# google/sbsim

Hardware: AMD Instinct MI355X
Metric: zone-updates/sec (env-steps/sec x 9 zones) at batch=64k buildings per GPU (higher is better)
Workload: dtype f64

## Files before the change

sbsim_amd/csrc/step_roll.hip:

```cpp
#include "step_roll_cfg.h"
#include "sweep_common.h"

namespace sb {
namespace {

using namespace sweep;
using namespace roll;

#ifndef SB_ONE_WAIT
#define SB_ONE_WAIT 1
#endif
constexpr int kWin = 63;
constexpr int kTS = 32;
constexpr int kSeamPad = 8;

struct PairBuf {
  d2 ud0, lr0, ud1, lr1;
  d2 A;
  d2 sm;
};

struct Acc {
  double cur;
  double neg;
  int sg;
  int tr, fin;
  double sre, sro;
};


template <int NR>
struct Ctx {
  const double *Arow;
  const double *Aext;
  const double *seam;
  const unsigned long long *cw;
  unsigned long long w, wn;
#ifdef SB_EXP_NOCOEF
  d2 kc;
#endif
};

template <int NR, int S>
__device__ __forceinline__ lds_d2 step_set(Ctx<NR> &x) {
  constexpr int j = S % NR;
  static_assert(NR % 8 == 0, "whole class words per period");
  if constexpr (j % 8 == 0) {
    x.w = x.wn;
    x.wn = x.cw[((j / 8 + 1) % (NR / 8)) * 64];
  }
  const unsigned h = j % 8 < 4 ? (unsigned)x.w : (unsigned)(x.w >> 32);
  unsigned off;
  if constexpr (j % 4 == 0) asm("v_lshlrev_b32_sdwa %0, 5, %1 dst_sel:DWORD dst_unused:UNUSED_PAD src0_sel:DWORD src1_sel:BYTE_0" : "=v"(off) : "v"(h));
  else if constexpr (j % 4 == 1) asm("v_lshlrev_b32_sdwa %0, 5, %1 dst_sel:DWORD dst_unused:UNUSED_PAD src0_sel:DWORD src1_sel:BYTE_1" : "=v"(off) : "v"(h));
  else if constexpr (j % 4 == 2) asm("v_lshlrev_b32_sdwa %0, 5, %1 dst_sel:DWORD dst_unused:UNUSED_PAD src0_sel:DWORD src1_sel:BYTE_2" : "=v"(off) : "v"(h));
  else asm("v_lshlrev_b32_sdwa %0, 5, %1 dst_sel:DWORD dst_unused:UNUSED_PAD src0_sel:DWORD src1_sel:BYTE_3" : "=v"(off) : "v"(h));
  return (lds_d2)off;
}

template <int NR, int S, bool SEAM, int NAR>
__device__ __forceinline__ void load_first(PairBuf &p, Ctx<NR> &x, const double (&Areg)[NAR]) {
#ifdef SB_EXP_NOCOEF
  p.ud0 = p.lr0 = x.kc;
  const lds_d2 ct = nullptr;
#else
  const lds_d2 ct = step_set<NR, S>(x);
  p.ud0 = ct[0];
#endif
#if defined(SB_EXP_ONECOEF)
  p.lr0 = p.ud0;
#elif !defined(SB_EXP_NOCOEF)
  p.lr0 = ct[1];
#endif
  constexpr int q = (S + 1) % NR, NL = lds_slots(NR), AS = a_stride(NR);
  static_assert(q % 2 == 0 && AS % 2 == 0, "pairs start at odd steps");
  if constexpr (q < AS) p.A = *(const d2 *)(x.Arow + q);
  else if constexpr (q < NL) p.A = *(const d2 *)(x.Aext + (q - AS));
  else p.A = d2{Areg[q - NL], Areg[q + 1 - NL]};
  if constexpr (SEAM && S >= kWin) p.sm = *(const d2 *)(x.seam + S);
  else p.sm = d2{0.0, 0.0};
}
template <int NR, int S>
__device__ __forceinline__ void load_second(PairBuf &p, Ctx<NR> &x) {
#ifdef SB_EXP_NOCOEF
  p.ud1 = p.lr1 = x.kc;
#else
  const lds_d2 ct = step_set<NR, S>(x);
  p.ud1 = ct[0];
#ifdef SB_EXP_ONECOEF
  p.lr1 = p.ud1;
#else
  p.lr1 = ct[1];
#endif
#endif
}

__device__ __forceinline__ void track(Acc &acc, double d) {
#ifdef SB_EXP_NOTRACK
  return;
#endif
  asm("v_max_f32 %0, %0, %1" : "+v"(acc.fin) : "v"(acc.tr));
  asm("v_max_f32_dpp %0, %0, |%1| wave_shr:1 row_mask:0xf bank_mask:0xf bound_ctrl:1" : "+v"(acc.tr) : "v"(__double2hiint(d)));
}

template <int NR, int S, bool EXACT, bool FREE = false>
__device__ __forceinline__ void step(double (&e)[NR], double (&bk)[kWin], d2 ud, d2 lr, double A,
                                     double sm, Acc &acc) {
  static_assert(S >= kWin, "the ramp-up has a step of its own: step_ramp");
  static_assert(!FREE || !EXACT, "free periods: the library's kernel");
  constexpr int r = S % NR, rm = (S + NR - 1) % NR, rp = (S + 1) % NR;
  const double Dn = wave_shift1<0x130, true>(e[rp], sm);
  double t;
  asm("v_fma_f64 %0, %1, %2, %3" : "=&v"(t) : "v"(ud.y), "v"(Dn), "v"(A));
  t = fma(lr.y, e[rp], t);
  const double U = wave_shift1<0x13c, false>(e[rm], 0.0);
  t = fma(lr.x, e[rm], t);
  const double nv = fma(ud.x, U, t);
#ifndef SB_EXP_NOSR
  if constexpr (S > kWin) {
    double &sr = (S - kWin - 1) % 2 == 0 ? acc.sre : acc.sro;
    sr = wave_shift1<0x138, true>(sr, U);
  }
#endif
  if constexpr (S < NR) {
    if constexpr (EXACT) acc.cur = fmax(acc.cur, fabs(nv - e[r]));
    else if constexpr (!FREE) track(acc, nv - e[r]);
    e[r] = nv;
  } else if constexpr (!EXACT) {
    constexpr int J = S - NR;
    track(acc, nv - e[r]);
#ifndef SB_EXP_NOCOPY
    if constexpr (!FREE) bk[J] = e[r];
#endif
    e[r] = nv;
  } else {
    constexpr int J = S - NR;
    const double d = nv - e[r];
    bk[J] = e[r];
    e[r] = nv;
    const double sd = __hiloint2double((__double2hiint(d) & 0x7fffffff) | acc.sg, __double2loint(d));
    acc.cur = fmax(acc.cur, sd);
    acc.neg = fmin(acc.neg, sd);
    if constexpr (J + 1 < kWin)
      acc.sg = __builtin_amdgcn_update_dpp(acc.sg, acc.sg, 0x138, 0xf, 0xf, false);
    asm volatile("" : "+v"(acc.cur), "+v"(acc.neg));
  }
}

template <int NR, int S, bool EXACT>
__device__ __forceinline__ void step_ramp(double (&e)[NR], d2 ud, d2 lr, double A, Acc &acc, bool started) {
  static_assert(S < kWin, "ramp-up steps only");
  constexpr int r = S % NR, rm = (S + NR - 1) % NR, rp = (S + 1) % NR;
  const double Dn = wave_shift1<0x130, false>(e[rp], 0.0);
  double t = fma(ud.y, Dn, A);
  t = fma(lr.y, e[rp], t);
  const double U = wave_shift1<0x13c, false>(e[rm], 0.0);
  t = fma(lr.x, e[rm], t);
  const double nv = fma(ud.x, U, t);
  const double sel = started ? nv : e[r];
  if constexpr (EXACT) {
    acc.cur = fmax(acc.cur, fabs(sel - e[r]));
  } else {
#ifndef SB_EXP_NOTRACK
    asm("v_max_f32_dpp %0, %0, |%1| wave_shr:1 row_mask:0xf bank_mask:0xf bound_ctrl:1" : "+v"(acc.tr) : "v"(__double2hiint(sel - e[r])));
#endif
  }
  e[r] = sel;
}

constexpr int kA0 = 8;
template <int NR, int NAR>
struct APass {
  const unsigned long long (&cw)[(NR + 7) / 8];
  unsigned tbase;
  double *Aw, *Ax;
  double (&Areg)[NAR];
  template <int J>
  __device__ __forceinline__ d2 fetch() const {
    static_assert(kTS * 8 == 256, "a class byte (class * 8) is the byte offset into ap[] and into g[]");
    const unsigned h = (J & 7) < 4 ? (unsigned)cw[J >> 3] : (unsigned)(cw[J >> 3] >> 32);
    unsigned ad;
    if constexpr ((J & 3) == 0) asm("v_add_u32_sdwa %0, %1, %2 dst_sel:DWORD dst_unused:UNUSED_PAD src0_sel:DWORD src1_sel:BYTE_0" : "=v"(ad) : "s"(tbase), "v"(h));
    else if constexpr ((J & 3) == 1) asm("v_add_u32_sdwa %0, %1, %2 dst_sel:DWORD dst_unused:UNUSED_PAD src0_sel:DWORD src1_sel:BYTE_1" : "=v"(ad) : "s"(tbase), "v"(h));
    else if constexpr ((J & 3) == 2) asm("v_add_u32_sdwa %0, %1, %2 dst_sel:DWORD dst_unused:UNUSED_PAD src0_sel:DWORD src1_sel:BYTE_2" : "=v"(ad) : "s"(tbase), "v"(h));
    else asm("v_add_u32_sdwa %0, %1, %2 dst_sel:DWORD dst_unused:UNUSED_PAD src0_sel:DWORD src1_sel:BYTE_3" : "=v"(ad) : "s"(tbase), "v"(h));
    const __attribute__((address_space(3))) double *tp = (const __attribute__((address_space(3))) double *)ad;
    return d2{tp[0], tp[kTS]};
  }
  template <int J>
  __device__ __forceinline__ void put(const d2 &pg, const double &ej) const {
    constexpr int q = (J + 1) % NR, NL = lds_slots(NR), AS = a_stride(NR);
    double av;
    asm("v_fma_f64 %0, %1, %2, %3" : "=v"(av) : "v"(pg.x), "v"(ej), "v"(pg.y));
    if constexpr (q < AS) Aw[q] = av;
    else if constexpr (q < NL) Ax[q - AS] = av;
    else Areg[q - NL] = av;
  }
};

#ifndef SB_DEPTH
#define SB_DEPTH 1
#endif
constexpr int kDepth = SB_DEPTH;
constexpr int kBufs = kDepth + 1;
constexpr int pair_buf(int S) { return ((S - 1) / 2) % kBufs; }

struct APrev {
  d2 v[3];
};

template <int NR, int S, int S1, bool WRAP, bool EXACT, bool APASS, bool FREE, int NAR>
__device__ __forceinline__ void roll_pairs(double (&e)[NR], double (&bk)[kWin], double (&Areg)[NAR],
                                           PairBuf (&pb)[kBufs], Ctx<NR> &x, Acc &acc, const APass<NR, NAR> &ap,
                                           const APrev pv = APrev{}) {
  if constexpr (S < S1) {
    static_assert(!APASS || S1 <= kWin, "the A pass belongs to the ramp-up");
    constexpr bool wrapped = WRAP && S + 2 * kDepth >= S1;
    constexpr int N = wrapped ? S + 2 * kDepth - NR : S + 2 * kDepth;
    PairBuf &cur = pb[pair_buf(S)], &nxt = pb[pair_buf(N)];
#if SB_ONE_WAIT
    if constexpr (S < kWin) asm volatile("" ::"v"(cur.ud0.x), "v"(cur.A.x), "v"(cur.ud1.x), "v"(cur.lr1.x));
    else asm volatile("" ::"v"(cur.ud0.x), "v"(cur.A.x), "v"(cur.sm.x), "v"(cur.ud1.x), "v"(cur.lr1.x));
    __builtin_amdgcn_sched_barrier(0);
#endif
    load_first<NR, N, !wrapped>(nxt, x, Areg);
    constexpr int j0 = kA0 + 3 * ((S - 1) / 2), jp = j0 - 3;
    static_assert(!APASS || (S % 2 == 1 && jp >= S + 2 * kDepth + 2), "a slot's A is written before the pair that reads it ahead");
    static_assert(!APASS || jp >= S + 2, "a slot still holds Tprev when its A is formed");
    static_assert(!APASS || S + 2 < S1 || j0 >= NR, "the ramp-up's last pair asks for no slot: no pair would form its A");
    if constexpr (APASS && S > 1) {
      if constexpr (jp < NR) ap.template put<jp < NR ? jp : 0>(pv.v[0], e[jp < NR ? jp : 0]);
      if constexpr (jp + 1 < NR) ap.template put<jp + 1 < NR ? jp + 1 : 0>(pv.v[1], e[jp + 1 < NR ? jp + 1 : 0]);
      if constexpr (jp + 2 < NR) ap.template put<jp + 2 < NR ? jp + 2 : 0>(pv.v[2], e[jp + 2 < NR ? jp + 2 : 0]);
    }
    bool m0 = false, m1 = false;
    if constexpr (S < kWin) m0 = lanes_upto<S < kWin ? S : 0>();
    if constexpr (S + 1 < kWin) m1 = lanes_upto<S + 1 < kWin ? S + 1 : 0>();
    APrev pa{{d2{0.0, 0.0}, d2{0.0, 0.0}, d2{0.0, 0.0}}};
    if constexpr (APASS && j0 < NR) pa.v[0] = ap.template fetch<j0 < NR ? j0 : 0>();
    if constexpr (APASS && j0 + 1 < NR) pa.v[1] = ap.template fetch<j0 + 1 < NR ? j0 + 1 : 0>();
    if constexpr (APASS && j0 + 2 < NR) pa.v[2] = ap.template fetch<j0 + 2 < NR ? j0 + 2 : 0>();
    __builtin_amdgcn_sched_barrier(0);
    if constexpr (S < kWin) step_ramp<NR, S, EXACT>(e, cur.ud0, cur.lr0, cur.A.x, acc, m0);
    else step<NR, S, EXACT, FREE>(e, bk, cur.ud0, cur.lr0, cur.A.x, cur.sm.x, acc);
    __builtin_amdgcn_sched_barrier(0);
    load_second<NR, N + 1>(nxt, x);
    __builtin_amdgcn_sched_barrier(0);
    if constexpr (S + 1 < kWin) step_ramp<NR, S + 1, EXACT>(e, cur.ud1, cur.lr1, cur.A.y, acc, m1);
    else step<NR, S + 1, EXACT, FREE>(e, bk, cur.ud1, cur.lr1, cur.A.y, cur.sm.y, acc);
    __builtin_amdgcn_sched_barrier(0);
    roll_pairs<NR, S + 2, S1, WRAP, EXACT, APASS, FREE>(e, bk, Areg, pb, x, acc, ap, pa);
  }
}

template <int NR, int J>
__device__ __forceinline__ void hand_over(double (&e)[NR], const double (&bk)[kWin], const unsigned long long (&zw)[NR / 8],
                                          double *tp, const double *np_, double *zrow) {
  static_assert(NR % 8 == 0, "whole zone words");
  if constexpr (J < NR) {
    if constexpr (J < kWin) e[J] = lanes_upto<J>() ? bk[J] : e[J];
    if constexpr (J + 1 < kWin) e[J + 1] = lanes_upto<J + 1>() ? bk[J + 1] : e[J + 1];
    const unsigned w = (J & 7) < 4 ? (unsigned)zw[J / 8] : (unsigned)(zw[J / 8] >> 32);
    const unsigned off0 = (w >> (8 * (J & 3))) & 0xffu, off1 = (w >> (8 * ((J + 1) & 3))) & 0xffu;
#ifndef SB_EXP_NOMEM
    __builtin_nontemporal_store(d2{e[J], e[J + 1]}, (d2 *)(tp + J * 64));
#endif
    __hip_atomic_fetch_add((double *)((char *)zrow + off0), e[J], __ATOMIC_RELAXED, __HIP_MEMORY_SCOPE_WORKGROUP);
    __hip_atomic_fetch_add((double *)((char *)zrow + off1), e[J + 1], __ATOMIC_RELAXED, __HIP_MEMORY_SCOPE_WORKGROUP);
#ifndef SB_EXP_NOMEM
    const d2 nv = __builtin_nontemporal_load((const d2 *)(np_ + J * 64));
    e[J] = nv.x;
    e[J + 1] = nv.y;
#endif
    if constexpr ((J & 7) == 6) __builtin_amdgcn_sched_barrier(0);
    hand_over<NR, J + 2>(e, bk, zw, tp, np_, zrow);
  }
}

template <int NR>
__device__ __forceinline__ void row63_to_tail(const double (&e)[NR], Acc &acc, int lane, double &U0, double &U1) {
  constexpr int last = (NR + kWin - 1) % NR;
  const double ul = wave_shift1<0x13c, false>(e[last], 0.0);
  double &sr = (NR - 1) % 2 == 0 ? acc.sre : acc.sro;
  sr = wave_shift1<0x138, true>(sr, ul);
  const int rev = (63 - lane) * 4;
  U0 = __hiloint2double(__builtin_amdgcn_ds_bpermute(rev, __double2hiint(acc.sre)),
                        __builtin_amdgcn_ds_bpermute(rev, __double2loint(acc.sre)));
  U1 = __hiloint2double(__builtin_amdgcn_ds_bpermute(rev, __double2hiint(acc.sro)),
                        __builtin_amdgcn_ds_bpermute(rev, __double2loint(acc.sro)));
}

extern __shared__ __attribute__((aligned(16))) double lds[];

template <int NR, bool EXACT>
__global__ void __launch_bounds__(64 * kWaves) __attribute__((amdgpu_waves_per_eu(1, 1))) k_sweep_roll(Dev a) {
  const int nB = a.redo_mode ? __builtin_amdgcn_readfirstlane(a.redo_ctr[0]) : a.B;
  if (nB == 0) return;
  const int lane = threadIdx.x & 63;
  const int wave = __builtin_amdgcn_readfirstlane((int)threadIdx.x >> 6);
  const int gw = (int)blockIdx.x * kWaves + wave;
  constexpr int kASlots = (NR + 7) / 8, kZSlots = NR / 8, kCW = NR / 8;
  static_assert((NR / 2) % kBufs == 0, "pair buffers rotate through a whole period: pair_buf() must not alias across the wrap");
  constexpr int kNL = lds_slots(NR), kAS = a_stride(NR), kNAR = NR - kNL > 0 ? NR - kNL : 2;

  double *tabc = lds;
  unsigned long long *ctab8 = (unsigned long long *)(lds + a.r_cmap);
  double *tmul = lds + a.r_cmap + kCW * 64;
  double *wl = tmul + a.tmul_doubles + (size_t)wave * a.lds_wave_doubles;
  double *tapg = wl;
  double *tE0 = wl + a.r_seam + 2;
  double *A = wl + a.r_A;
  for (int i = threadIdx.x; i < a.lds_reg_bytes / 8; i += blockDim.x) lds[i] = 0.0;
  __syncthreads();
  for (int i = threadIdx.x; i < 4 * kTS; i += blockDim.x) tabc[i] = i < 4 * a.ncset ? a.csetab[i] : 0.0;
  for (int i = threadIdx.x; i < kCW * 64; i += blockDim.x) ctab8[i] = a.cmapS[i];
  for (int i = threadIdx.x; i < a.tmul_doubles; i += blockDim.x) tmul[i] = a.tmulS[i];
  if (lane < kTS) tapg[lane] = lane <= a.ncls ? a.ctab[lane * 8 + 4] : 0.0;
  __syncthreads();

  const sb_params &p = a.p;
  const int R = lane;
  constexpr int RS = 64;
  if ((unsigned)(size_t)(__attribute__((address_space(3))) double *)tabc != 0u) __builtin_trap();
  Ctx<NR> x;
  x.Arow = A + (size_t)R * kAS;
  x.Aext = A + 64 * kAS + (size_t)R * (kNL - kAS);
  x.seam = tE0 - kWin;
  x.cw = ctab8 + lane;
  x.w = x.wn = 0;
#ifdef SB_EXP_NOCOEF
  x.kc = d2{0.2 + 1e-9 * opaque(lane), 0.2};
#endif
  const bool tactive = tail_col<NR>(lane, 0) >= 0;
  const int tc0 = tactive ? tail_col<NR>(lane, 0) : 0;
  const int tcw = tactive ? tc0 : -2;
  int tset[kTailMax], tcls8[kTailMax];
#pragma unroll
  for (int t = 0; t < kTailMax; ++t) {
    tset[t] = (a.ncset - 1) * 32 * 0x10001;
    tcls8[t] = (8 * a.ncls) | ((8 * a.ncls) << 8);
    if (t < a.T && tactive) {
      const int c0 = tc0, c1 = tc0 + 1;
      tset[t] = ((int)a.tcset[t * NR + c0] << 2) | ((int)a.tcset[t * NR + c1] << 18);
      tcls8[t] = (int)a.tcls[t * NR + c0] | ((int)a.tcls[t * NR + c1] << 8);
    }
  }
  const unsigned long long *amap = a.amapS + lane;
  const unsigned long long *zmap = a.zmapS + lane;

#ifdef SB_PHASE_STAMPS
#define SB_STAMP(i) do { if (a.dbg && gw == 0 && iter == 10 && lane == 0) a.dbg[i] = (long long)__builtin_readcyclecounter(); } while (0)
#else
#define SB_STAMP(i) do { } while (0)
#endif

  double e[NR];
  double nx_g = 0.0, nx_tail[kTailMax][2] = {{0.0, 0.0}, {0.0, 0.0}}, nx_tnow = 0.0, nx_lo = 0.0, nx_hi = 0.0;
#define SB_LOAD_AUX(bb)                                                                         \
  do {                                                                                          \
    nx_tnow = a.bld[(bb)].t_now;                                                                \
    nx_lo = a.scal[(size_t)(bb) * kNScal + 16];                                                 \
    nx_hi = a.scal[(size_t)(bb) * kNScal + 17];                                                 \
    nx_g = a.gtabg[(size_t)(bb) * kTS + (opaque(lane) & (kTS - 1))];  \
    const double *tt_ = a.temp + (size_t)(bb) * a.state_doubles + NR * 64;                      \
    _Pragma("unroll") for (int t = 0; t < kTailMax; ++t)                                        \
      _Pragma("unroll") for (int k = 0; k < 2; ++k)                                             \
        if (t < a.T) nx_tail[t][k] = tt_[t * NR + tc0 + k];                                     \
  } while (0)
  auto building = [&](int s) { return a.redo_mode ? __builtin_amdgcn_readfirstlane(a.redo_list[s]) : s; };
  const int b_first = gw < nB ? building(gw) : 0;
  if (gw < nB) {
    const double *tp_ = a.temp + (size_t)b_first * a.state_doubles;
#pragma unroll
    for (int j = 0; j < NR; j += 2) {
      const d2 v = __builtin_nontemporal_load((const d2 *)(tp_ + j * 64 + 2 * R));
      e[j] = v.x;
      e[j + 1] = v.y;
    }
    SB_LOAD_AUX(b_first);
  }
  unsigned long long amapw[kASlots];
#define SB_LOAD_AMAP(g0, g1)                                                                    \
  do {                                                                                          \
    const int o_ = opaque(0);                                                                   \
    _Pragma("unroll") for (int g = (g0); g < (g1); ++g) amapw[g] = amap[o_ + g * 64];           \
  } while (0)
  constexpr int kAHalf = kASlots / 2;
  SB_LOAD_AMAP(0, kASlots);
  int iter = 0;
  for (int s = gw, sn = 0, b = b_first, bn = 0; s < nB; s = sn, b = bn, ++iter) {
    int nb = 0;
    if (lane == 0) nb = atomicAdd(a.next_b, 1);
    SB_STAMP(0);
    x.wn = x.cw[0];
    __builtin_amdgcn_sched_barrier(0);
    const double t_now = nx_tnow;
    const double ring_d = a.n_ring > 0 ? fmax(fabs(t_now - nx_lo), fabs(t_now - nx_hi)) : 0.0;
    if (lane < kTS) tapg[kTS + opaque(lane)] = nx_g;
    double tv[kTailMax][2];
#pragma unroll
    for (int t = 0; t < kTailMax; ++t)
#pragma unroll
      for (int k = 0; k < 2; ++k) tv[t][k] = tactive ? nx_tail[t][k] : 0.0;
    *(d2 *)(tE0 + opaque(tcw)) = d2{tv[0][0], tv[0][1]};
    __builtin_amdgcn_wave_barrier();
    __builtin_amdgcn_sched_barrier(0);
    SB_STAMP(1);
    double At[kTailMax][2] = {{0.0, 0.0}, {0.0, 0.0}};
    if constexpr (!EXACT) {
      const double *pg[kTailMax][2];
#pragma unroll
      for (int t = 0; t < kTailMax; ++t)
#pragma unroll
        for (int k = 0; k < 2; ++k) pg[t][k] = (const double *)((const char *)tapg + ((opaque(tcls8[t]) >> (8 * k)) & 0xff));
      double tap[kTailMax][2], tg[kTailMax][2];
#pragma unroll
      for (int t = 0; t < kTailMax; ++t)
#pragma unroll
        for (int k = 0; k < 2; ++k) { tap[t][k] = pg[t][k][0]; tg[t][k] = pg[t][k][kTS]; }
#pragma unroll
      for (int t = 0; t < kTailMax; ++t)
#pragma unroll
        for (int k = 0; k < 2; ++k) At[t][k] = fma(tap[t][k], tv[t][k], tg[t][k]);
    } else {
#pragma unroll
      for (int t = 0; t < kTailMax; ++t)
#pragma unroll
        for (int k = 0; k < 2; ++k)
          if (t < a.T && tactive) {
            const int c8 = (opaque(tcls8[t]) >> (8 * k)) & 0xff;
            const double *pg = (const double *)((const char *)tapg + c8);
            At[t][k] = fma(pg[0], tv[t][k], pg[kTS]);
          }
    }

    double Areg[kNAR];
    Areg[0] = 0.0;
    const APass<NR, kNAR> ap{amapw, (unsigned)(size_t)(__attribute__((address_space(3))) double *)tapg, A + (size_t)R * kAS,
                             A + 64 * kAS + (size_t)R * (kNL - kAS), Areg};
    {
      static_assert(kA0 == 8 && kA0 + 3 * ((kWin - 3) / 2) >= NR, "the ramp-up's pairs but the last one reach the last slot");
      const d2 g0 = ap.template fetch<0>(), g1 = ap.template fetch<1>(), g2 = ap.template fetch<2>(), g3 = ap.template fetch<3>(),
               g4 = ap.template fetch<4>(), g5 = ap.template fetch<5>(), g6 = ap.template fetch<6>(), g7 = ap.template fetch<7>();
      __builtin_amdgcn_sched_barrier(0);
      ap.template put<0>(g0, e[0]); ap.template put<1>(g1, e[1]); ap.template put<2>(g2, e[2]); ap.template put<3>(g3, e[3]);
      ap.template put<4>(g4, e[4]); ap.template put<5>(g5, e[5]); ap.template put<6>(g6, e[6]); ap.template put<7>(g7, e[7]);
    }
    __builtin_amdgcn_wave_barrier();
    __builtin_amdgcn_sched_barrier(0);
    SB_STAMP(2);

    int n_sweeps = 0, converged = 0, redo = 0;
    double bk[kWin];
    {
      PairBuf pb[kBufs];
      Acc acc;
      acc.cur = 0.0; acc.neg = 0.0; acc.sg = lane == 0 ? (int)0x80000000 : 0;
      acc.tr = acc.fin = 0;
      acc.sre = acc.sro = 0.0;
      {
        const lds_d2 ct = step_set<NR, 0>(x);
        const d2 ud = ct[0], lr = ct[1];
        load_first<NR, 1, true>(pb[pair_buf(1)], x, Areg);
        load_second<NR, 2>(pb[pair_buf(1)], x);
        if constexpr (kDepth > 1) {
          load_first<NR, 3, true>(pb[pair_buf(3)], x, Areg);
          load_second<NR, 4>(pb[pair_buf(3)], x);
        }
        static_assert(kDepth <= 2, "initial fill of the pair buffers");
        step_ramp<NR, 0, EXACT>(e, ud, lr, x.Arow[1], acc, lanes_upto<0>());
      }
      __builtin_amdgcn_sched_barrier(0);
      roll_pairs<NR, 1, kWin, false, EXACT, true, false>(e, bk, Areg, pb, x, acc, ap);
#ifndef SB_STAMP_NEXT
      SB_STAMP(15);
#endif
#pragma nounroll
      for (;;) {
        __builtin_amdgcn_sched_barrier(0);
#ifdef SB_PHASE_STAMPS
#ifndef SB_STAMP_SWEEP
#define SB_STAMP_SWEEP 1
#endif
#define SB_STAMP2(i) do { if (a.dbg && gw == 0 && iter == 10 && sweep_idx == SB_STAMP_SWEEP && lane == 0) a.dbg[i] = (long long)__builtin_readcyclecounter(); } while (0)
        const int sweep_idx = n_sweeps;
#ifdef SB_STAMP_NEXT
        if (a.dbg && gw == 0 && iter == 10 && sweep_idx == SB_STAMP_SWEEP + 1 && lane == 0) a.dbg[15] = (long long)__builtin_readcyclecounter();
#endif
#else
#define SB_STAMP2(i) do { } while (0)
#endif
        if constexpr (!EXACT) {
          if (a.roll_free) {
            const int thr_top = __double2hiint(p.conv_threshold);
            int top = wave_max_i32(acc.tr);
            if (n_sweeps == 0) top = max(top, __double2hiint(ring_d));
#pragma nounroll
            while (top > thr_top && n_sweeps + 1 < p.iter_limit) {
              __builtin_amdgcn_sched_barrier(0);
              roll_pairs<NR, kWin, NR + kWin, true, false, false, true>(e, bk, Areg, pb, x, acc, ap);
              double F0, F1;
              row63_to_tail<NR>(e, acc, lane, F0, F1);
              tail_pass_static_values<NR>(a.T, tmul + opaque(tc0), tE0 + opaque(tcw), F0, F1, tv, tset, At);
              pb[pair_buf(kWin)].sm = *(const d2 *)(x.seam + kWin);
              if constexpr (kDepth > 1) pb[pair_buf(kWin + 2)].sm = *(const d2 *)(x.seam + kWin + 2);
              ++n_sweeps;
              acc.fin = 0;
              acc.tr = lanes_upto<62>() ? acc.tr : 0;
              top = wave_max_i32(acc.tr);
              __builtin_amdgcn_sched_barrier(0);
            }
          }
        }
        SB_STAMP2(10);
        roll_pairs<NR, kWin, NR + kWin, true, EXACT, false, false>(e, bk, Areg, pb, x, acc, ap);
        SB_STAMP2(11);
        double U0, U1;
        row63_to_tail<NR>(e, acc, lane, U0, U1);
        SB_STAMP2(12);
        const double dt_ = tail_pass_static<NR>(a.T, tmul + opaque(tc0), tE0 + opaque(tcw), U0, U1, tv, tset, At);

        SB_STAMP2(13);
        if constexpr (EXACT) {
          double md = wave_max(fmax(acc.cur, dt_));
          if (n_sweeps == 0) md = fmax(md, ring_d);
          ++n_sweeps;
          converged = md <= p.conv_threshold;
        } else {
          asm("v_max_f32 %0, %0, %1" : "+v"(acc.fin) : "v"(acc.tr));
          int m_hi = max(__builtin_amdgcn_readlane(acc.fin, 63), wave_max_i32(__double2hiint(dt_)));
          if (n_sweeps == 0) m_hi = max(m_hi, __double2hiint(ring_d));
          const int thr_hi = __double2hiint(p.conv_threshold);
          ++n_sweeps;
          acc.fin = 0;
          acc.tr = lanes_upto<62>() ? acc.tr : 0;
          const bool undecided = m_hi == thr_hi || (a.dbg_redo_mod > 0 && b % a.dbg_redo_mod == 0);
          if (m_hi <= thr_hi && undecided) { redo = 1; break; }
          converged = m_hi < thr_hi;
        }
        SB_STAMP2(14);
#ifdef SB_EXP_DESYNC
        if (n_sweeps >= 1 + (int)(((unsigned)b * 2654435761u >> 13) % 9u)) break;
#else
        if (converged || n_sweeps >= p.iter_limit) break;
#endif
        pb[pair_buf(kWin)].sm = *(const d2 *)(x.seam + kWin);
        if constexpr (kDepth > 1) pb[pair_buf(kWin + 2)].sm = *(const d2 *)(x.seam + kWin + 2);
        acc.cur = -acc.neg;
        acc.neg = 0.0;
        acc.sg = lane == 0 ? (int)0x80000000 : 0;
      }
    }
    __builtin_amdgcn_sched_barrier(0);
    SB_STAMP(3);
    sn = a.sweep_wgs + __builtin_amdgcn_readfirstlane(nb);
    bn = sn < nB ? building(sn) : 0;
    if (sn < nB) SB_LOAD_AUX(bn);
    SB_LOAD_AMAP(0, kAHalf);
    __builtin_amdgcn_sched_barrier(0);
    SB_STAMP(4);

    double *zs = A;
    const int ZRS = a.ZRS;
    {
      unsigned long long zw[kZSlots];
      const unsigned long long *zm = zmap + opaque(0);
#pragma unroll
      for (int g = 0; g < kZSlots; ++g) zw[g] = zm[g * 64];
      __builtin_amdgcn_sched_barrier(0);
      double *tp = redo ? a.redo_scratch + (size_t)gw * a.state_doubles : a.temp + (size_t)b * a.state_doubles;
      double *Ttail = tp + NR * 64;
      double *zrow = zs + (size_t)opaque(R) * ZRS;
      for (int z = 0; z <= a.Z; ++z) zrow[z] = 0.0;
      __builtin_amdgcn_wave_barrier();
#pragma unroll
      for (int t = 0; t < kTailMax; ++t)
        if (t < a.T && tactive) {
          *(d2 *)(Ttail + t * NR + tc0) = d2{tv[t][0], tv[t][1]};
          zrow[a.Z] += tv[t][0] + tv[t][1];
        }
      const double *np_ = a.temp + (size_t)(sn < nB ? bn : b) * a.state_doubles;
      static_assert(RS == 64, "hand_over: slot stride");
      hand_over<NR, 0>(e, bk, zw, tp + 2 * R, np_ + 2 * R, zrow);
    }
    __builtin_amdgcn_sched_barrier(0);
    SB_STAMP(5);
    SB_LOAD_AMAP(kAHalf, kASlots);
    __builtin_amdgcn_sched_barrier(0);
    SB_STAMP(6);
    __builtin_amdgcn_wave_barrier();
    SB_STAMP(7);

    {
      double gacc = 0.0;
      for (int zb = 0; zb <= a.Z; zb += 16) {
        const int zz = zb + (lane >> 2), g = lane & 3;
        const double *zr = zs + (size_t)g * ZRS + (zz <= a.Z ? zz : a.Z);
        double part[RS / 4];
#pragma unroll
        for (int k = 0; k < RS / 4; ++k) part[k] = zr[(size_t)4 * k * ZRS];
        double v = 0.0;
#pragma unroll
        for (int k = 0; k < RS / 4; ++k) v += part[k];
        if (zz > a.Z) v = 0.0;
        v += dpp_or_zero<0xB1, 0xf>(v);
        v += dpp_or_zero<0x4E, 0xf>(v);
        if (g == 0 && zz < a.Z && !redo) a.zsum[(size_t)b * a.Z + zz] = v;
        if (g == 0 && zz <= a.Z) gacc += v;
      }
      const double gsum = wave_sum(gacc);
      if (lane == 0 && !redo) {
        a.gsum[b] = gsum + a.n_ring_f64 * t_now;
        a.nsw[b] = n_sweeps | (converged << 16);
      }
      if (lane == 0 && redo) a.redo_list[atomicAdd(a.redo_ctr, 1)] = b;
      SB_STAMP(8);
#ifdef SB_PHASE_STAMPS
      if (a.dbg && gw == 0 && iter == 10 && lane == 0) a.dbg[9] = n_sweeps;
#endif
    }
  }
#undef SB_STAMP
#undef SB_LOAD_AUX
#undef SB_LOAD_AMAP
}

}

int sweep_roll_redo_workgroups() { return 8; }

namespace {

template <int NR>
int prepare(const Dev &d) {
  const int e = (int)hipFuncSetAttribute((const void *)k_sweep_roll<NR, false>, hipFuncAttributeMaxDynamicSharedMemorySize,
                                         d.lds_reg_bytes);
  if (e != (int)hipSuccess) return e;
  return (int)hipFuncSetAttribute((const void *)k_sweep_roll<NR, true>, hipFuncAttributeMaxDynamicSharedMemorySize,
                                  d.lds_reg_bytes);
}

template <int NR>
int launch(const Dev &d, hipStream_t stream) {
  const dim3 grid((d.sweep_wgs + kWaves - 1) / kWaves), block(64 * kWaves);
  if (d.roll_exact) {
    hipLaunchKernelGGL((k_sweep_roll<NR, true>), grid, block, (size_t)d.lds_reg_bytes, stream, d);
    return (int)hipGetLastError();
  }
  hipLaunchKernelGGL((k_sweep_roll<NR, false>), grid, block, (size_t)d.lds_reg_bytes, stream, d);
  Dev r = d;
  r.redo_mode = 1;
  r.next_b = d.redo_ctr + 1;
  r.sweep_wgs = sweep_roll_redo_workgroups() * kWaves;
  hipLaunchKernelGGL((k_sweep_roll<NR, true>), dim3(sweep_roll_redo_workgroups()), block, (size_t)d.lds_reg_bytes, stream, r);
  return (int)hipGetLastError();
}

}

int prepare_sweep_roll(const Dev &d) {
  if (d.NR == 96) return prepare<96>(d);
  if (d.NR == 88) return prepare<88>(d);
  if (d.NR == 80) return prepare<80>(d);
  if (d.NR == 72) return prepare<72>(d);
  if (d.NR == 64) return prepare<64>(d);
  return (int)hipErrorInvalidValue;
}

int launch_sweep_roll(const Dev &d, hipStream_t stream) {
  if (d.NR == 96) return launch<96>(d, stream);
  if (d.NR == 88) return launch<88>(d, stream);
  if (d.NR == 80) return launch<80>(d, stream);
  if (d.NR == 72) return launch<72>(d, stream);
  if (d.NR == 64) return launch<64>(d, stream);
  return (int)hipErrorInvalidValue;
}

}
```

sbsim_amd/csrc/step_roll_cfg.h:

```cpp
#pragma once

namespace sb {
namespace roll {

constexpr int kSlotCounts[] = {64, 72, 80, 88, 96};
constexpr int lds_slots(int NR) { return NR >= 72 ? 72 : ((NR / 2) % 2 ? NR : NR + 2); }
constexpr int a_stride(int NR) { return NR >= 72 ? 70 : ((NR / 2) % 2 ? NR : NR + 2); }
constexpr int kWaves = 4;
constexpr int tail_row(int NR) { return NR + 4; }
constexpr int tail_mul_doubles(int NR, int T) { return T > 0 ? (4 * T + 2) * (NR / 2) : 0; }

}
}
```

sbsim_amd/csrc/sweep_common.h:

```cpp
#pragma once

#include <type_traits>

#include "sb_device.h"

namespace sb {
namespace sweep {

constexpr int kTailMax = 2;

__device__ __forceinline__ int opaque(int v) {
  asm volatile("" : "+v"(v));
  return v;
}
__device__ __forceinline__ int opaque_s(int v) {
  asm volatile("" : "+s"(v));
  return v;
}

template <int I, int N, class F>
__device__ __forceinline__ void static_for(F &&f) {
  if constexpr (I < N) {
    f(std::integral_constant<int, I>{});
    static_for<I + 1, N>(f);
  }
}

template <int J>
__device__ __forceinline__ bool lanes_upto() {
  unsigned long long m;
  asm volatile("s_bfm_b64 %0, %1, 0" : "=s"(m) : "n"(J + 1));
  return __builtin_amdgcn_inverse_ballot_w64(m);
}

template <int CTRL, bool SEAM>
__device__ __forceinline__ double wave_shift1(double x, double old) {
  int lo, hi;
  if (SEAM) {
    lo = __builtin_amdgcn_update_dpp(__double2loint(old), __double2loint(x), CTRL, 0xf, 0xf, false);
    hi = __builtin_amdgcn_update_dpp(__double2hiint(old), __double2hiint(x), CTRL, 0xf, 0xf, false);
  } else {
    lo = __builtin_amdgcn_update_dpp(0, __double2loint(x), CTRL, 0xf, 0xf, true);
    hi = __builtin_amdgcn_update_dpp(0, __double2hiint(x), CTRL, 0xf, 0xf, true);
  }
  return __hiloint2double(hi, lo);
}

typedef double d2 __attribute__((ext_vector_type(2)));
typedef const d2 __attribute__((address_space(3))) *lds_d2;
typedef volatile int __attribute__((address_space(3))) *lds_vi;

template <int CTRL, int ROW_MASK>
__device__ __forceinline__ void scan_step(double &a, double &q) {
  const double one = 1.0;
  const int alo = __builtin_amdgcn_update_dpp(__double2loint(one), __double2loint(a), CTRL, ROW_MASK, 0xf, false);
  const int ahi = __builtin_amdgcn_update_dpp(__double2hiint(one), __double2hiint(a), CTRL, ROW_MASK, 0xf, false);
  const int qlo = __builtin_amdgcn_update_dpp(0, __double2loint(q), CTRL, ROW_MASK, 0xf, false);
  const int qhi = __builtin_amdgcn_update_dpp(0, __double2hiint(q), CTRL, ROW_MASK, 0xf, false);
  const double as = __hiloint2double(ahi, alo), qs = __hiloint2double(qhi, qlo);
  q = fma(a, qs, q);
  a = a * as;
}
__device__ __forceinline__ void affine_scan(double &a, double &q) {
  scan_step<0x111, 0xf>(a, q);
  scan_step<0x112, 0xf>(a, q);
  scan_step<0x114, 0xf>(a, q);
  scan_step<0x118, 0xf>(a, q);
  scan_step<0x142, 0xa>(a, q);
  scan_step<0x143, 0xc>(a, q);
}

template <int NR>
__device__ __forceinline__ int tail_col(int lane, int k) { return 2 * (lane - (64 - NR / 2)) + k; }

template <int NR>
__device__ __forceinline__ double tail_pass(int T, bool active, double *tE0c, double U0, double U1,
                                            double (&tv)[kTailMax][2], const int (&tset)[kTailMax],
                                            const double (&At)[kTailMax][2]) {
  static_assert(NR % 2 == 0 && NR <= 128, "two columns per lane");
  double dmax = 0.0;
#pragma unroll
  for (int t = 0; t < kTailMax; ++t) {
    if (t < T) {
      const lds_d2 s0 = (lds_d2)(unsigned)(tset[t] & 0xffff), s1 = (lds_d2)((unsigned)tset[t] >> 16);
      const d2 ud0 = s0[0], lr0 = s0[1], ud1 = s1[0], lr1 = s1[1];
      const double old0 = tv[t][0], old1 = tv[t][1];
      const double R1 = wave_shift1<0x130, false>(old0, 0.0);
      const double D0 = t + 1 < T ? tv[t + 1 < kTailMax ? t + 1 : t][0] : 0.0, D1 = t + 1 < T ? tv[t + 1 < kTailMax ? t + 1 : t][1] : 0.0;
      const double q0 = fma(ud0.x, U0, fma(lr0.y, old1, fma(ud0.y, D0, At[t][0])));
      const double q1 = fma(ud1.x, U1, fma(lr1.y, R1, fma(ud1.y, D1, At[t][1])));
      double a = lr1.x * lr0.x, Q = fma(lr1.x, q0, q1);
      affine_scan(a, Q);
      const double xl = wave_shift1<0x138, false>(Q, 0.0);
      const double x0 = fma(lr0.x, xl, q0);
      if (active) {
        dmax = fmax(dmax, fmax(fabs(x0 - old0), fabs(Q - old1)));
        tv[t][0] = x0;
        tv[t][1] = Q;
        if (t == 0) *(d2 *)tE0c = d2{x0, Q};
      }
      U0 = x0;
      U1 = Q;
    }
  }
  return dmax;
}


template <int CTRL, int ROW_MASK>
__device__ __forceinline__ void scan_level(double &q, double A, double &qs) {
  const int lo = __builtin_amdgcn_update_dpp(__double2loint(qs), __double2loint(q), CTRL, ROW_MASK, 0xf, true);
  const int hi = __builtin_amdgcn_update_dpp(__double2hiint(qs), __double2hiint(q), CTRL, ROW_MASK, 0xf, true);
  qs = __hiloint2double(hi, lo);
  q = fma(A, qs, q);
}

template <int NR, bool MEASURE>
__device__ __forceinline__ double tail_pass_static_impl(int T, const double *tm, double *tE0c, double U0, double U1,
                                                        double (&tv)[kTailMax][2], const int (&tset)[kTailMax],
                                                        const double (&At)[kTailMax][2]) {
  static_assert(NR % 2 == 0 && NR <= 128, "two columns per lane");
  constexpr int n = NR / 2;
  double dmax = 0.0;
#pragma unroll
  for (int t = 0; t < kTailMax; ++t) {
    if (t < T) {
      const lds_d2 s0 = (lds_d2)(unsigned)(tset[t] & 0xffff), s1 = (lds_d2)((unsigned)tset[t] >> 16);
      const d2 ud0 = s0[0], lr0 = s0[1], ud1 = s1[0], lr1 = s1[1];
      const d2 A12 = *(const d2 *)(tm + 4 * n * t), A34 = *(const d2 *)(tm + 4 * n * t + 2 * n);
      const double old0 = tv[t][0], old1 = tv[t][1];
      const double R1 = wave_shift1<0x130, false>(old0, 0.0);
      double q0 = At[t][0], q1 = At[t][1];
      if (t + 1 < T) {
        q0 = fma(ud0.y, tv[t + 1 < kTailMax ? t + 1 : t][0], q0);
        q1 = fma(ud1.y, tv[t + 1 < kTailMax ? t + 1 : t][1], q1);
      }
      q0 = fma(ud0.x, U0, fma(lr0.y, old1, q0));
      q1 = fma(ud1.x, U1, fma(lr1.y, R1, q1));
      double Q = fma(lr1.x, q0, q1), qs = 0.0;
      scan_level<0x111, 0xf>(Q, lr1.x * lr0.x, qs);
      scan_level<0x112, 0xf>(Q, A12.x, qs);
      scan_level<0x114, 0xf>(Q, A12.y, qs);
      scan_level<0x118, 0xf>(Q, A34.x, qs);
      scan_level<0x142, 0xa>(Q, A34.y, qs);
      scan_level<0x143, 0xc>(Q, tm[4 * n * T + t], qs);
      const double xl = wave_shift1<0x138, false>(Q, 0.0);
      const double x0 = fma(lr0.x, xl, q0);
      if constexpr (MEASURE) dmax = fmax(dmax, fmax(fabs(x0 - old0), fabs(Q - old1)));
      tv[t][0] = x0;
      tv[t][1] = Q;
      if (t == 0) *(d2 *)tE0c = d2{x0, Q};
      U0 = x0;
      U1 = Q;
    }
  }
  return dmax;
}
template <int NR>
__device__ __forceinline__ double tail_pass_static(int T, const double *tm, double *tE0c, double U0, double U1,
                                                   double (&tv)[kTailMax][2], const int (&tset)[kTailMax],
                                                   const double (&At)[kTailMax][2]) {
  return tail_pass_static_impl<NR, true>(T, tm, tE0c, U0, U1, tv, tset, At);
}
template <int NR>
__device__ __forceinline__ void tail_pass_static_values(int T, const double *tm, double *tE0c, double U0, double U1,
                                                        double (&tv)[kTailMax][2], const int (&tset)[kTailMax],
                                                        const double (&At)[kTailMax][2]) {
  (void)tail_pass_static_impl<NR, false>(T, tm, tE0c, U0, U1, tv, tset, At);
}

}
}
```

Before: 305.9 million.

## Fold tail seam contribution into LDS A row for folded steps

For steps whose A term lives in LDS, the tail pass now folds the seam coupling (coefficient times the tail's first-row value) directly into the A entry of lane 63's row, instead of storing a separate seam value that each step adds via a DPP shift. Folded steps then skip the per-step seam load and use a plain wave shift with zero fill. After each tail pass the affected A pairs are reloaded from LDS. This moves a per-step cost into a once-per-sweep fixup, at the price of extra packed control bits, table lookups and more complex bookkeeping in the tail pass.

New measurement: 308.1 million, median of 6. About the same (+0.7%).

```diff
diff --git a/sbsim_amd/csrc/step_roll.hip b/sbsim_amd/csrc/step_roll.hip
--- a/sbsim_amd/csrc/step_roll.hip
+++ b/sbsim_amd/csrc/step_roll.hip
@@ -77,8 +77,15 @@
   if constexpr (q < AS) p.A = *(const d2 *)(x.Arow + q);
   else if constexpr (q < NL) p.A = *(const d2 *)(x.Aext + (q - AS));
   else p.A = d2{Areg[q - NL], Areg[q + 1 - NL]};
-  if constexpr (SEAM && S >= kWin) p.sm = *(const d2 *)(x.seam + S);
+  if constexpr (SEAM && S >= kWin && !fold_step(NR, S)) p.sm = *(const d2 *)(x.seam + S);
   else p.sm = d2{0.0, 0.0};
+}
+template <int NR, int S>
+__device__ __forceinline__ void reload_A(PairBuf &p, const Ctx<NR> &x) {
+  constexpr int q = (S + 1) % NR, AS = a_stride(NR);
+  static_assert(S % 2 == 1 && fold_step(NR, S), "a folded pair: its A is in LDS");
+  if constexpr (q < AS) p.A = *(const d2 *)(x.Arow + q);
+  else p.A = *(const d2 *)(x.Aext + (q - AS));
 }
 template <int NR, int S>
 __device__ __forceinline__ void load_second(PairBuf &p, Ctx<NR> &x) {
@@ -109,9 +116,10 @@
   static_assert(S >= kWin, "the ramp-up has a step of its own: step_ramp");
   static_assert(!FREE || !EXACT, "free periods: the library's kernel");
   constexpr int r = S % NR, rm = (S + NR - 1) % NR, rp = (S + 1) % NR;
-  const double Dn = wave_shift1<0x130, true>(e[rp], sm);
+  const double Dn = fold_step(NR, S) ? wave_shift1<0x130, false>(e[rp], 0.0) : wave_shift1<0x130, true>(e[rp], sm);
   double t;
-  asm("v_fma_f64 %0, %1, %2, %3" : "=&v"(t) : "v"(ud.y), "v"(Dn), "v"(A));
+  if constexpr (FREE && fold_step(NR, S)) t = fma(ud.y, Dn, A);
+  else asm("v_fma_f64 %0, %1, %2, %3" : "=&v"(t) : "v"(ud.y), "v"(Dn), "v"(A));
   t = fma(lr.y, e[rp], t);
   const double U = wave_shift1<0x13c, false>(e[rm], 0.0);
   t = fma(lr.x, e[rm], t);
@@ -219,7 +227,7 @@
     constexpr int N = wrapped ? S + 2 * kDepth - NR : S + 2 * kDepth;
     PairBuf &cur = pb[pair_buf(S)], &nxt = pb[pair_buf(N)];
 #if SB_ONE_WAIT
-    if constexpr (S < kWin) asm volatile("" ::"v"(cur.ud0.x), "v"(cur.A.x), "v"(cur.ud1.x), "v"(cur.lr1.x));
+    if constexpr (S < kWin || fold_step(NR, S)) asm volatile("" ::"v"(cur.ud0.x), "v"(cur.A.x), "v"(cur.ud1.x), "v"(cur.lr1.x));
     else asm volatile("" ::"v"(cur.ud0.x), "v"(cur.A.x), "v"(cur.sm.x), "v"(cur.ud1.x), "v"(cur.lr1.x));
     __builtin_amdgcn_sched_barrier(0);
 #endif
@@ -344,6 +352,14 @@
       tset[t] = ((int)a.tcset[t * NR + c0] << 2) | ((int)a.tcset[t * NR + c1] << 18);
       tcls8[t] = (int)a.tcls[t * NR + c0] | ((int)a.tcls[t * NR + c1] << 8);
     }
+  }
+  if (a.T > 0 && tactive) {
+    const unsigned char *cb = (const unsigned char *)a.cmapS;
+    const int s0 = (tc0 + kWin) % NR, s1 = (tc0 + kWin + 1) % NR, q = s1;
+    const int set0 = cb[((s0 >> 3) * 64 + 63) * 8 + (s0 & 7)], set1 = cb[((s1 >> 3) * 64 + 63) * 8 + (s1 & 7)];
+    static_assert(kTS <= 32, "five bits per coefficient set");
+    tcls8[0] |= TailFold::pack0(set0, set1, fold_pos(NR, q));
+    tcls8[1] |= TailFold::pack1(fold_pos(NR, q) ? fold_dest(NR, q) : 0);
   }
   const unsigned long long *amap = a.amapS + lane;
   const unsigned long long *zmap = a.zmapS + lane;
@@ -472,6 +488,19 @@
       }
       __builtin_amdgcn_sched_barrier(0);
       roll_pairs<NR, 1, kWin, false, EXACT, true, false>(e, bk, Areg, pb, x, acc, ap);
+      static_assert(kA0 + 3 * ((kWin - 3) / 2) - 1 >= NR - 1, "the ramp-up's last pair forms A of the last slot: lane 63's row is whole before the first fold");
+      {
+        __builtin_amdgcn_sched_barrier(0);
+        const TailFold tf = TailFold::unpack(tcls8[0], tcls8[1], tabc, A);
+        double *tE0c = tE0 + opaque(tcw), *src = tf.on ? tf.dst : tE0c;
+        const d2 P = *(const d2 *)src;
+        const double b0 = *tf.bd0, b1 = *tf.bd1;
+        *(d2 *)tE0c = P;
+        *(d2 *)src = tf.on ? d2{fma(b0, tv[0][0], P.x), fma(b1, tv[0][1], P.y)} : P;
+        reload_A<NR, kWin>(pb[pair_buf(kWin)], x);
+        if constexpr (kDepth > 1) reload_A<NR, kWin + 2>(pb[pair_buf(kWin + 2)], x);
+        __builtin_amdgcn_sched_barrier(0);
+      }
 #ifndef SB_STAMP_NEXT
       SB_STAMP(15);
 #endif
@@ -501,9 +530,9 @@
               roll_pairs<NR, kWin, NR + kWin, true, false, false, true>(e, bk, Areg, pb, x, acc, ap);
               double F0, F1;
               row63_to_tail<NR>(e, acc, lane, F0, F1);
-              tail_pass_static_values<NR>(a.T, tmul + opaque(tc0), tE0 + opaque(tcw), F0, F1, tv, tset, At);
-              pb[pair_buf(kWin)].sm = *(const d2 *)(x.seam + kWin);
-              if constexpr (kDepth > 1) pb[pair_buf(kWin + 2)].sm = *(const d2 *)(x.seam + kWin + 2);
+              tail_pass_static_values<NR>(a.T, tmul + opaque(tc0), tE0 + opaque(tcw), F0, F1, tv, tset, At, tcls8[0], tcls8[1], tabc, A);
+              reload_A<NR, kWin>(pb[pair_buf(kWin)], x);
+              if constexpr (kDepth > 1) reload_A<NR, kWin + 2>(pb[pair_buf(kWin + 2)], x);
               ++n_sweeps;
               acc.fin = 0;
               acc.tr = lanes_upto<62>() ? acc.tr : 0;
@@ -518,7 +547,7 @@
         double U0, U1;
         row63_to_tail<NR>(e, acc, lane, U0, U1);
         SB_STAMP2(12);
-        const double dt_ = tail_pass_static<NR>(a.T, tmul + opaque(tc0), tE0 + opaque(tcw), U0, U1, tv, tset, At);
+        const double dt_ = tail_pass_static<NR>(a.T, tmul + opaque(tc0), tE0 + opaque(tcw), U0, U1, tv, tset, At, tcls8[0], tcls8[1], tabc, A);
 
         SB_STAMP2(13);
         if constexpr (EXACT) {
@@ -544,8 +573,8 @@
 #else
         if (converged || n_sweeps >= p.iter_limit) break;
 #endif
-        pb[pair_buf(kWin)].sm = *(const d2 *)(x.seam + kWin);
-        if constexpr (kDepth > 1) pb[pair_buf(kWin + 2)].sm = *(const d2 *)(x.seam + kWin + 2);
+        reload_A<NR, kWin>(pb[pair_buf(kWin)], x);
+        if constexpr (kDepth > 1) reload_A<NR, kWin + 2>(pb[pair_buf(kWin + 2)], x);
         acc.cur = -acc.neg;
         acc.neg = 0.0;
         acc.sg = lane == 0 ? (int)0x80000000 : 0;
diff --git a/sbsim_amd/csrc/step_roll_cfg.h b/sbsim_amd/csrc/step_roll_cfg.h
--- a/sbsim_amd/csrc/step_roll_cfg.h
+++ b/sbsim_amd/csrc/step_roll_cfg.h
@@ -6,6 +6,11 @@
 constexpr int kSlotCounts[] = {64, 72, 80, 88, 96};
 constexpr int lds_slots(int NR) { return NR >= 72 ? 72 : ((NR / 2) % 2 ? NR : NR + 2); }
 constexpr int a_stride(int NR) { return NR >= 72 ? 70 : ((NR / 2) % 2 ? NR : NR + 2); }
+constexpr bool fold_pos(int NR, int q) { return q + 1 < lds_slots(NR); }
+constexpr bool fold_step(int NR, int S) { return fold_pos(NR, ((S % 2 ? S : S - 1) + 1) % NR); }
+constexpr int fold_dest(int NR, int q) {
+  return q < a_stride(NR) ? 63 * a_stride(NR) + q : 64 * a_stride(NR) + 63 * (lds_slots(NR) - a_stride(NR)) + (q - a_stride(NR));
+}
 constexpr int kWaves = 4;
 constexpr int tail_row(int NR) { return NR + 4; }
 constexpr int tail_mul_doubles(int NR, int T) { return T > 0 ? (4 * T + 2) * (NR / 2) : 0; }
diff --git a/sbsim_amd/csrc/sweep_common.h b/sbsim_amd/csrc/sweep_common.h
--- a/sbsim_amd/csrc/sweep_common.h
+++ b/sbsim_amd/csrc/sweep_common.h
@@ -107,6 +107,19 @@
 }
 
 
+struct TailFold {
+  bool on;
+  const double *bd0, *bd1;
+  double *dst;
+  static __device__ __forceinline__ int pack0(int set0, int set1, bool on) { return (set0 | (set1 << 5) | (on ? 1 << 10 : 0)) << 16; }
+  static __device__ __forceinline__ int pack1(int dst_doubles) { return (dst_doubles >> 1) << 16; }
+  static __device__ __forceinline__ TailFold unpack(int w0, int w1, const double *tab, double *A) {
+    const unsigned u0 = (unsigned)opaque(w0) >> 16, u1 = (unsigned)opaque(w1) >> 16;
+    return TailFold{(u0 & 0x400u) != 0, (const double *)((const char *)tab + ((u0 & 31u) << 5) + 8),
+                    (const double *)((const char *)tab + (u0 & 0x3e0u) + 8), A + 2 * u1};
+  }
+};
+
 template <int CTRL, int ROW_MASK>
 __device__ __forceinline__ void scan_level(double &q, double A, double &qs) {
   const int lo = __builtin_amdgcn_update_dpp(__double2loint(qs), __double2loint(q), CTRL, ROW_MASK, 0xf, true);
@@ -118,7 +131,7 @@
 template <int NR, bool MEASURE>
 __device__ __forceinline__ double tail_pass_static_impl(int T, const double *tm, double *tE0c, double U0, double U1,
                                                         double (&tv)[kTailMax][2], const int (&tset)[kTailMax],
-                                                        const double (&At)[kTailMax][2]) {
+                                                        const double (&At)[kTailMax][2], int fw0, int fw1, const double *ftab, double *fA) {
   static_assert(NR % 2 == 0 && NR <= 128, "two columns per lane");
   constexpr int n = NR / 2;
   double dmax = 0.0;
@@ -149,7 +162,14 @@
       if constexpr (MEASURE) dmax = fmax(dmax, fmax(fabs(x0 - old0), fabs(Q - old1)));
       tv[t][0] = x0;
       tv[t][1] = Q;
-      if (t == 0) *(d2 *)tE0c = d2{x0, Q};
+      if (t == 0) {
+        __builtin_amdgcn_sched_barrier(0);
+        const TailFold tf = TailFold::unpack(fw0, fw1, ftab, fA);
+        const d2 P = *(const d2 *)tE0c;
+        const double b0 = *tf.bd0, b1 = *tf.bd1;
+        const d2 Af = d2{fma(b0, x0, P.x), fma(b1, Q, P.y)};
+        *(d2 *)(tf.on ? tf.dst : tE0c) = tf.on ? Af : d2{x0, Q};
+      }
       U0 = x0;
       U1 = Q;
     }
@@ -159,14 +179,14 @@
 template <int NR>
 __device__ __forceinline__ double tail_pass_static(int T, const double *tm, double *tE0c, double U0, double U1,
                                                    double (&tv)[kTailMax][2], const int (&tset)[kTailMax],
-                                                   const double (&At)[kTailMax][2]) {
-  return tail_pass_static_impl<NR, true>(T, tm, tE0c, U0, U1, tv, tset, At);
+                                                   const double (&At)[kTailMax][2], int fw0, int fw1, const double *ftab, double *fA) {
+  return tail_pass_static_impl<NR, true>(T, tm, tE0c, U0, U1, tv, tset, At, fw0, fw1, ftab, fA);
 }
 template <int NR>
 __device__ __forceinline__ void tail_pass_static_values(int T, const double *tm, double *tE0c, double U0, double U1,
                                                         double (&tv)[kTailMax][2], const int (&tset)[kTailMax],
-                                                        const double (&At)[kTailMax][2]) {
-  (void)tail_pass_static_impl<NR, false>(T, tm, tE0c, U0, U1, tv, tset, At);
+                                                        const double (&At)[kTailMax][2], int fw0, int fw1, const double *ftab, double *fA) {
+  (void)tail_pass_static_impl<NR, false>(T, tm, tE0c, U0, U1, tv, tset, At, fw0, fw1, ftab, fA);
 }
 
 }
```
